# rensortino/DDP-Tutorial

Measured on AMD Instinct MI355X. Metric: images/sec (whole node), ResNet-18 CIFAR-10, higher is better.
Workload: dtype bf16; 1 GPU; model=resnet18, global_batch=8192, image_size=32, num_classes=10, parallelism=dp1, sync_bn=False, hip_graph=False

## Files before the change

mi355x/csrc/conv_mfma.hip:

```cpp
#include "conv_internal.h"

typedef __attribute__((ext_vector_type(8))) _Float16 half8;
typedef __attribute__((ext_vector_type(16))) float f32x16;

namespace {

template <typename T16>
struct Mfma32 {};
template <>
struct Mfma32<__hip_bfloat16> {
  static DEV_INLINE f32x16 run(short8 a, short8 b, f32x16 c) {
    return __builtin_amdgcn_mfma_f32_32x32x16_bf16(a, b, c, 0, 0, 0);
  }
};
template <>
struct Mfma32<__half> {
  static DEV_INLINE f32x16 run(short8 a, short8 b, f32x16 c) {
    return __builtin_amdgcn_mfma_f32_32x32x16_f16((half8)a, (half8)b, c, 0, 0,
                                                  0);
  }
};

struct Sc8 {
  float4v s0, s1, h0, h1;
};

DEV_INLINE Sc8 sc8_load(const float* __restrict__ asc,
                        const float* __restrict__ ash, int c) {
  Sc8 r;
  r.s0 = *reinterpret_cast<const float4v*>(asc + c);
  r.s1 = *reinterpret_cast<const float4v*>(asc + c + 4);
  r.h0 = *reinterpret_cast<const float4v*>(ash + c);
  r.h1 = *reinterpret_cast<const float4v*>(ash + c + 4);
  return r;
}

template <typename T16>
DEV_INLINE short8 scale8(short8 v, const Sc8& sc) {
  short8 o;
#pragma unroll
  for (int u = 0; u < 4; ++u) {
    const float f = s16_to_f32<T16>(v[u]) * sc.s0[u] + sc.h0[u];
    o[u] = f32_to_s16<T16>(fmaxf(f, 0.f));
  }
#pragma unroll
  for (int u = 0; u < 4; ++u) {
    const float f = s16_to_f32<T16>(v[4 + u]) * sc.s1[u] + sc.h1[u];
    o[4 + u] = f32_to_s16<T16>(fmaxf(f, 0.f));
  }
  return o;
}

// ... 107 lines not shown
    if (cc_i == 0) {
      bool va = m_ok;
      long ioff = 0;
      if constexpr (TRANS) {
        const int ph = ih0 + pad - r_;
        const int qw = iw0 + pad - s_;
        const int pp = ph / stride, qq = qw / stride;
        va = va && ph >= 0 && qw >= 0 && (ph % stride) == 0 &&
             (qw % stride) == 0 && pp < Hi && qq < Wi;
        if (va) ioff = (((long)n_ * Hi + pp) * Wi + qq) * CI;
      } else {
        const int ih = ih0 + r_;
        const int iw = iw0 + s_;
        va = va && (unsigned)ih < (unsigned)Hi && (unsigned)iw < (unsigned)Wi;
        if (va) ioff = (((long)n_ * Hi + ih) * Wi + iw) * CI;
      }
      va_tap = va;
      ioff_tap = ioff;
    }
    if (++cc_i == cchunks) {
      cc_i = 0;
      if (++s_i == S) {
        s_i = 0;
        ++r_i;
      }
    }
    const bool va = va_tap;
    const long ioff = ioff_tap;
    const T16* xp = va ? in + ioff + c0 + sa_c : zpage;
#pragma unroll
    for (int i = 0; i < 4; ++i)
      sa[i] = *reinterpret_cast<const short8*>(xp + (va ? 8 * i : 0));
    if constexpr (SCALED) {
      if (va) {
#pragma unroll
        for (int i = 0; i < 4; ++i)
          sa[i] = scale8<T16>(sa[i],
                              sc8_load(asc, ash, c0 + sa_c + 8 * i));
      }
    }
    const T16* wp = wrow + (long)(r_ * S + s_) * b_rs_stride + c0;
#pragma unroll
    for (int i = 0; i < EPT / 8; ++i)
      sb[i] = *reinterpret_cast<const short8*>(wp + 8 * i);
  };

  auto stage = [&]() {
    T16* ldsA = lds;
    T16* ldsB = lds + BM * LDK;
    short* pa = reinterpret_cast<short*>(ldsA + sa_m * LDK + sa_c);
#pragma unroll
    for (int i = 0; i < 4; ++i)
      *reinterpret_cast<short8*>(pa + 8 * i) = sa[i];
    short* pb = reinterpret_cast<short*>(ldsB + sb_n * LDK + sb_c);
#pragma unroll
    for (int i = 0; i < EPT / 8; ++i)
      *reinterpret_cast<short8*>(pb + 8 * i) = sb[i];
  };

  load_step(0);
  for (int j = 0; j < ksteps; ++j) {
    __syncthreads();
    stage();
    __syncthreads();
    if (j + 1 < ksteps) load_step(j + 1);
    const T16* ldsA = lds;
    const T16* ldsB = lds + BM * LDK;
#pragma unroll
    for (int kk = 0; kk < BK; kk += 16) {
      const short8 af = *reinterpret_cast<const short8*>(
          ldsA + (wm + li) * LDK + kk + kh * 8);
#pragma unroll
      for (int tnt = 0; tnt < NT; ++tnt) {
        const short8 bf = *reinterpret_cast<const short8*>(
            ldsB + (tnt * 32 + li) * LDK + kk + kh * 8);
        acc[tnt] = Mfma32<T16>::run(af, bf, acc[tnt]);
      }
    }
  }

  float bv[NT];
  float ssum[NT] = {}, ssq[NT] = {};
#pragma unroll
  for (int tnt = 0; tnt < NT; ++tnt)
    bv[tnt] = has_bias ? bias[k0 + tnt * 32 + li] : 0.f;
#pragma unroll
  for (int reg = 0; reg < 16; ++reg) {
    const int row = (reg & 3) + 8 * (reg >> 2) + 4 * kh;
    const long m_out = bm0 + wm + row;
    if (m_out < Mtot) {
#pragma unroll
      for (int tnt = 0; tnt < NT; ++tnt) {
        float v = acc[tnt][reg] + bv[tnt];
        if constexpr (ADDIN)
          v += F16<T16>::to_f32(addin[m_out * KO + k0 + tnt * 32 + li]);
        if (act == 1) v = fmaxf(v, 0.f);
        if (stats_slab) {
          ssum[tnt] += v;
          ssq[tnt] += v * v;
        }
        out[m_out * KO + k0 + tnt * 32 + li] = F16<T16>::from_f32(v);
      }
    }
  }
  if (stats_slab) {
    constexpr int BNTC = NT * 32;
#pragma unroll
    for (int tnt = 0; tnt < NT; ++tnt) {
      ssum[tnt] += __shfl_xor(ssum[tnt], 32, 64);
      ssq[tnt] += __shfl_xor(ssq[tnt], 32, 64);
    }
    float* lsum = reinterpret_cast<float*>(lds);
    __syncthreads();
    if (kh == 0) {
#pragma unroll
      for (int tnt = 0; tnt < NT; ++tnt) {
        lsum[wave * 2 * BNTC + tnt * 32 + li] = ssum[tnt];
        lsum[wave * 2 * BNTC + BNTC + tnt * 32 + li] = ssq[tnt];
      }
    }
    __syncthreads();
    float* slab =
        stats_slab + ((long)blockIdx.y * gridDim.x + blockIdx.x) * 2 * BNTC;
    for (int t = tid; t < 2 * BNTC; t += 256)
      slab[t] = lsum[t] + lsum[2 * BNTC + t] + lsum[4 * BNTC + t] +
                lsum[6 * BNTC + t];
  }
}

__global__ void conv_stats_partial(const float* __restrict__ slab,
                                   float* __restrict__ out, int gx, int bnt2,
                                   int bpb) {
  const int by = blockIdx.y;
  const int t = threadIdx.x;
  if (t >= bnt2) return;
  const int b0 = blockIdx.x * bpb;
  const int b1 = min(gx, b0 + bpb);
  float acc = 0.f;
  for (int bx = b0; bx < b1; ++bx)
    acc += slab[((long)by * gx + bx) * bnt2 + t];
  out[((long)by * gridDim.x + blockIdx.x) * bnt2 + t] = acc;
}

__global__ void conv_stats_reduce(const float* __restrict__ slab,
                                  float* __restrict__ stats, int gx, int bnt2,
                                  int C, int bx_per_block) {
  const int by = blockIdx.y;
  const int t = threadIdx.x;
  if (t >= bnt2) return;
  float acc = 0.f;
  const int b0 = blockIdx.x * bx_per_block;
  const int b1 = min(gx, b0 + bx_per_block);
  for (int bx = b0; bx < b1; ++bx)
    acc += slab[((long)by * gx + bx) * bnt2 + t];
  const int bnt = bnt2 / 2;
  const int h = t / bnt;
  const int c = by * bnt + (t % bnt);
  stats[h * C + c] = acc;
}

template <typename T16, int NT, bool ADDIN = false>
__global__ __launch_bounds__(256, 2) void conv_dgrad_s2_gemm(
    const T16* __restrict__ dy,
    const T16* __restrict__ wflip,
    const T16* __restrict__ zpage,
    const T16* __restrict__ addin,
    T16* __restrict__ dx,
    const int N, const int P, const int Q, const int KO, const int CI,
    const int H, const int W, const int R, const int S, const int pad) {
  __shared__ T16 lds[BM * LDK + NT * 32 * LDK];
  const int tid = threadIdx.x;
// ... 28 lines not shown
  constexpr int TPR = 256 / BNT;
  constexpr int EPT = BK / TPR;
  const int sb_n = tid / TPR;
  const int sb_c = (tid % TPR) * EPT;

  const int wave = tid >> 6;
  const int lane = tid & 63;
  const int li = lane & 31;
  const int kh = lane >> 5;
  const int wm = wave * 32;
  f32x16 acc[NT] = {};
  short8 sa[4], sb[EPT / 8];

  int cc_i = 0, s_i = 0, r_i = 0;
  bool va_tap = false;
  long ioff_tap = 0, woff_tap = 0;
  auto load_step = [&](int j) {
    (void)j;
    const int c0 = cc_i * BK;
    if (cc_i == 0) {
      const int s_ = s0 + 2 * s_i;
      const int r_ = r0 + 2 * r_i;
      const int dh = ih_ + pad - r_;
      const int dw_ = iw_ + pad - s_;
      const int pp = dh >> 1, qq = dw_ >> 1;
      va_tap = m_ok && dh >= 0 && dw_ >= 0 && pp < P && qq < Q;
      ioff_tap = (((long)n_ * P + pp) * Q + qq) * KO;
      woff_tap = ((long)r_ * S + s_) * CI * (long)KO;
    }
    if (++cc_i == cchunks) {
      cc_i = 0;
      if (++s_i == ns) {
        s_i = 0;
        ++r_i;
      }
    }
    const bool va = va_tap;
    const T16* xp = va ? dy + ioff_tap + c0 + sa_c : zpage;
#pragma unroll
    for (int i = 0; i < 4; ++i)
      sa[i] = *reinterpret_cast<const short8*>(xp + (va ? 8 * i : 0));
    const T16* wp = wflip + woff_tap + (long)(k0 + sb_n) * KO + c0 + sb_c;
#pragma unroll
    for (int i = 0; i < EPT / 8; ++i)
      sb[i] = *reinterpret_cast<const short8*>(wp + 8 * i);
  };
  auto stage = [&]() {
    T16* ldsA = lds;
    T16* ldsB = lds + BM * LDK;
    short* pa_ = reinterpret_cast<short*>(ldsA + sa_m * LDK + sa_c);
#pragma unroll
    for (int i = 0; i < 4; ++i)
      *reinterpret_cast<short8*>(pa_ + 8 * i) = sa[i];
    short* pb_ = reinterpret_cast<short*>(ldsB + sb_n * LDK + sb_c);
#pragma unroll
    for (int i = 0; i < EPT / 8; ++i)
      *reinterpret_cast<short8*>(pb_ + 8 * i) = sb[i];
  };

  if (ksteps > 0) {
    load_step(0);
    for (int j = 0; j < ksteps; ++j) {
      __syncthreads();
      stage();
      __syncthreads();
      if (j + 1 < ksteps) load_step(j + 1);
      const T16* ldsA = lds;
      const T16* ldsB = lds + BM * LDK;
#pragma unroll
      for (int kk = 0; kk < BK; kk += 16) {
        const short8 af = *reinterpret_cast<const short8*>(
            ldsA + (wm + li) * LDK + kk + kh * 8);
#pragma unroll
        for (int tnt = 0; tnt < NT; ++tnt) {
          const short8 bf = *reinterpret_cast<const short8*>(
              ldsB + (tnt * 32 + li) * LDK + kk + kh * 8);
          acc[tnt] = Mfma32<T16>::run(af, bf, acc[tnt]);
        }
      }
    }
  }

  const long m_base = bm0 + wm;
  const int HaWa = Ha * Wa;
  int nn0 = 0, rem0 = 0;
  if (m_base < Mc) {
    nn0 = (int)(m_base / HaWa);
    rem0 = (int)(m_base % HaWa);
  }
#pragma unroll
  for (int reg = 0; reg < 16; ++reg) {
    const int row = (reg & 3) + 8 * (reg >> 2) + 4 * kh;
    const long m_out = m_base + row;
    if (m_out < Mc) {
      int nn = nn0, rem = rem0 + row;
      while (rem >= HaWa) {
        rem -= HaWa;
        ++nn;
      }
      const int ih = 2 * (rem / Wa) + pa;
      const int iw = 2 * (rem - (rem / Wa) * Wa) + pb;
      const long off = (((long)nn * H + ih) * W + iw) * CI;
#pragma unroll
      for (int tnt = 0; tnt < NT; ++tnt) {
        float v = acc[tnt][reg];
        if constexpr (ADDIN)
          v += F16<T16>::to_f32(addin[off + k0 + tnt * 32 + li]);
        dx[off + k0 + tnt * 32 + li] = F16<T16>::from_f32(v);
      }
    }
  }
}

}

void stats_slab_reduce(at::Tensor slab, at::Tensor stats, int gx, int bnt2,
                       int C) {
  const int by = (int)(slab.numel() / ((long)gx * bnt2));
  if (gx > 4096) {
    const int bpb1 = (int)cdiv_l(gx, 1024);
    const int gx2 = (int)cdiv_l(gx, bpb1);
    auto l2 = at::empty({(long)by * gx2 * bnt2}, slab.options());
    launch256(conv_stats_partial, dim3(gx2, by), 0, slab.data_ptr<float>(),
              l2.data_ptr<float>(), gx, bnt2, bpb1);
    slab = l2;
    gx = gx2;
  }
  if (gx > 64) {
    const int bpb2 = (int)cdiv_l(gx, 64);
    const int gx3 = (int)cdiv_l(gx, bpb2);
    auto l3 = at::empty({(long)by * gx3 * bnt2}, slab.options());
    launch256(conv_stats_partial, dim3(gx3, by), 0, slab.data_ptr<float>(),
              l3.data_ptr<float>(), gx, bnt2, bpb2);
    slab = l3;
    gx = gx3;
  }
  launch256(conv_stats_reduce, dim3(1, by), 0, slab.data_ptr<float>(),
            stats.data_ptr<float>(), gx, bnt2, C, gx);
}

constexpr int PCS = 72;

template <typename T16, bool TRANS, bool ADDIN = false, bool SCALED = false>
__global__ __launch_bounds__(256, 2) void conv_patch_gemm(
    const T16* __restrict__ in,
    const T16* __restrict__ wgt,
    const float* __restrict__ bias,
    const T16* __restrict__ addin,
    const float* __restrict__ asc,
    const float* __restrict__ ash,
    T16* __restrict__ out,
    float* __restrict__ stats_slab,
    const int N, const int Hi, const int Wi, const int CI, const int KO,
    const long b_row_stride, const long b_rs_stride, const int act,
    const int has_bias, const int NR) {
  extern __shared__ __attribute__((aligned(16))) char psmem[];
  T16* patch = reinterpret_cast<T16*>(psmem);
  T16* zstub = patch + (long)NR * (Wi + 2) * PCS;
  T16* ldsB = zstub + PCS;

  const int tid = threadIdx.x;
  const long Mtot = (long)N * Hi * Wi;
  const int Wo = Wi, Ho = Hi;
  const long bm0 = (long)blockIdx.x * 128;
  const int k0 = blockIdx.y * 64;
  const long gr0 = bm0 / Wo - 1;

  const int wave = tid >> 6;
  const int lane = tid & 63;
  const int li = lane & 31;
  const int kh = lane >> 5;
  const int wm = wave * 32;

  const long m_lane = bm0 + wm + li;
  const long grl = m_lane / Wo;
  const int p_lane = (int)(grl % Ho);
  const int prow = (int)(grl - gr0);
  const int pcol = (int)(m_lane - grl * Wo) + 1;
  const bool m_ok = m_lane < Mtot;
  const long lane_base = ((long)prow * (Wi + 2) + pcol) * PCS;

  if (tid < 64) zstub[tid] = T16{};

  const int cchunks = CI / BK;
  f32x16 acc[2] = {};

  const int sb_n = tid >> 2;
  const int sb_c = (tid & 3) * 16;
  const T16* wrowB = wgt + (long)(k0 + sb_n) * b_row_stride + sb_c;
  short8 breg[2];
  auto load_b = [&](int tap, int cc) {
    const T16* wp = wrowB + (long)tap * b_rs_stride + cc * BK;
    breg[0] = *reinterpret_cast<const short8*>(wp);
    breg[1] = *reinterpret_cast<const short8*>(wp + 8);
  };
  auto stage_b = [&]() {
    short* pb = reinterpret_cast<short*>(ldsB + sb_n * LDK + sb_c);
    *reinterpret_cast<short8*>(pb) = breg[0];
    *reinterpret_cast<short8*>(pb + 8) = breg[1];
  };

  load_b(0, 0);

  for (int cc = 0; cc < cchunks; ++cc) {
    __syncthreads();
    const int ngroups = NR * (Wi + 2) * (BK / 8);
    for (int i0f = tid; i0f < ngroups; i0f += 4 * 256) {
      const T16* srcs[4];
      short8 vals[4];
      int dsts[4], gs[4];
      bool ok[4];
#pragma unroll
      for (int b = 0; b < 4; ++b) {
        const int i = i0f + b * 256;
        const int g = i % (BK / 8);
        const int ce = i / (BK / 8);
        const int col = ce % (Wi + 2);
        const int row = ce / (Wi + 2);
        const long gr = gr0 + row;
        const int iw = col - 1;
        gs[b] = g;
        dsts[b] = i < ngroups ? (row * (Wi + 2) + col) * PCS + g * 8 : -1;
        ok[b] = i < ngroups && gr >= 0 && gr < (long)N * Ho &&
                (unsigned)iw < (unsigned)Wi;
        const long nn = ok[b] ? gr / Ho : 0;
        const long pp = ok[b] ? gr % Ho : 0;
        srcs[b] = ok[b]
                      ? in + ((nn * Hi + pp) * Wi + iw) * CI + cc * BK + g * 8
                      : zstub;
      }
#pragma unroll
      for (int b = 0; b < 4; ++b)
        vals[b] = *reinterpret_cast<const short8*>(srcs[b]);
#pragma unroll
      for (int b = 0; b < 4; ++b) {
        if (dsts[b] < 0) break;
        short8 v = vals[b];
        if (!ok[b]) v = short8{};
        if constexpr (SCALED) {
          if (ok[b])
            v = scale8<T16>(v, sc8_load(asc, ash, cc * BK + gs[b] * 8));
        }
        *reinterpret_cast<short8*>(patch + dsts[b]) = v;
      }
    }
    __syncthreads();

#pragma unroll
    for (int r = 0; r < 3; ++r) {
      const int pv = TRANS ? p_lane + 1 - r : p_lane + r - 1;
      const bool rv = m_ok && (unsigned)pv < (unsigned)Ho;
#pragma unroll
      for (int s = 0; s < 3; ++s) {
        const int tap = r * 3 + s;
        const long off = TRANS
                             ? ((long)(1 - r) * (Wi + 2) + (1 - s)) * PCS
                             : ((long)(r - 1) * (Wi + 2) + (s - 1)) * PCS;
        const T16* abase = rv ? patch + lane_base + off : zstub;
        __syncthreads();
        stage_b();
        __syncthreads();
        if (tap < 8)
          load_b(tap + 1, cc);
        else if (cc + 1 < cchunks)
          load_b(0, cc + 1);
#pragma unroll
        for (int kk = 0; kk < 4; ++kk) {
          const short8 af = *reinterpret_cast<const short8*>(
              abase + kk * 16 + kh * 8);
          const short8 b0 = *reinterpret_cast<const short8*>(
              ldsB + li * LDK + kk * 16 + kh * 8);
          const short8 b1 = *reinterpret_cast<const short8*>(
              ldsB + (32 + li) * LDK + kk * 16 + kh * 8);
          acc[0] = Mfma32<T16>::run(af, b0, acc[0]);
          acc[1] = Mfma32<T16>::run(af, b1, acc[1]);
        }
      }
    }
  }

  float bv[2];
  bv[0] = has_bias ? bias[k0 + li] : 0.f;
  bv[1] = has_bias ? bias[k0 + 32 + li] : 0.f;
  float ssum[2] = {}, ssq[2] = {};
#pragma unroll
  for (int reg = 0; reg < 16; ++reg) {
    const int row = (reg & 3) + 8 * (reg >> 2) + 4 * kh;
    const long m_out = bm0 + wm + row;
    if (m_out < Mtot) {
#pragma unroll
      for (int t2 = 0; t2 < 2; ++t2) {
        float v = acc[t2][reg] + bv[t2];
        if constexpr (ADDIN)
          v += F16<T16>::to_f32(addin[m_out * KO + k0 + t2 * 32 + li]);
        if (act == 1) v = fmaxf(v, 0.f);
        if (stats_slab) {
          ssum[t2] += v;
          ssq[t2] += v * v;
        }
        out[m_out * KO + k0 + t2 * 32 + li] = F16<T16>::from_f32(v);
      }
    }
  }
  if (stats_slab) {
#pragma unroll
    for (int t2 = 0; t2 < 2; ++t2) {
      ssum[t2] += __shfl_xor(ssum[t2], 32, 64);
      ssq[t2] += __shfl_xor(ssq[t2], 32, 64);
    }
    float* lsum = reinterpret_cast<float*>(psmem);
    __syncthreads();
    if (kh == 0) {
#pragma unroll
      for (int t2 = 0; t2 < 2; ++t2) {
        lsum[wave * 128 + t2 * 32 + li] = ssum[t2];
        lsum[wave * 128 + 64 + t2 * 32 + li] = ssq[t2];
      }
    }
    __syncthreads();
    float* slab =
        stats_slab + ((long)blockIdx.y * gridDim.x + blockIdx.x) * 2 * 64;
    for (int t = tid; t < 2 * 64; t += 256)
      slab[t] = lsum[t] + lsum[128 + t] + lsum[256 + t] + lsum[384 + t];
  }
}


namespace {

constexpr int WGM = 64;
constexpr int LDM = 72;

template <typename T16, int KT, bool SCALED = false, bool KMIN = false>
__global__ __launch_bounds__(256, SCALED ? 4 : 2) void conv_wgrad_mfma_kernel(
    const T16* __restrict__ x,
    const T16* __restrict__ dy,
    const float* __restrict__ asc,
    const float* __restrict__ ash,
    float* __restrict__ dw,
    const int N, const int Hi, const int Wi, const int CI, const int KO,
    const int Ho, const int Wo, const int R, const int S, const int stride,
    const int pad, const long m_per_chunk, const int nchunks) {
  __shared__ T16 lds[(KT + 64) * LDM];

  const int tid = threadIdx.x;
  const long Mtot = (long)N * Ho * Wo;
  const int k0 = blockIdx.x * KT;
  const int cchunks = CI / BK;
  const int c0 = (blockIdx.y % cchunks) * BK;
  const int s_ = (blockIdx.y / cchunks) % S;
  const int r_ = blockIdx.y / (cchunks * S);
  const long m_begin = (long)blockIdx.z * m_per_chunk;
  const long m_end = min(Mtot, m_begin + m_per_chunk);

  const bool do_dy = tid < 2 * KT;
  const bool do_x = KT == 64 ? tid >= 128 : tid < 128;
  const int t = do_dy ? tid : 0;
  constexpr int KG = KT / 8;
  const int sm = KMIN ? (t / KG) * 4 : (t & 15) * 4;
  const int sk = KMIN ? (t % KG) * 8 : (t >> 4) * 8;
  const int tx = tid & 127;
  const int smx = KMIN ? (tx >> 3) * 4 : (tx & 15) * 4;
  const int skx = KMIN ? (tx & 7) * 8 : (tx >> 4) * 8;

  const int wave = tid >> 6;
  const int lane = tid & 63;
  const int li = lane & 31;
  const int kh = lane >> 5;
  constexpr int NJ = KT / 64;
// ... 861 lines not shown
  at::Tensor zp = conv_zero_page(in);
  at::Tensor slab;
  if (present(stats))
    slab = at::empty({(long)grid.y * grid.x * 2 * nt * 32},
                     in.options().dtype(at::kFloat));
  DISPATCH_16(in, T16, {
    auto go = [&](auto kern) {
      launch256(kern, grid, 0, (const T16*)in.data_ptr(),
                (const T16*)wgt.data_ptr(), f32_or_null(bias),
                (const T16*)zp.data_ptr(),
                present(addin) ? (const T16*)addin.data_ptr() : nullptr, asc,
                ash, (T16*)out.data_ptr(), f32_or_null(slab), N, Hi, Wi, CI,
                KO, Ho, Wo, R, S, stride, pad, b_row_stride, b_rs_stride, act,
                present(bias));
    };
    if (genc)
      go(conv_gather_gemm<T16, false, true, 2>);
    else
      pick<4, 2>(nt, [&](auto NT) {
        if (trans)
          pick<true, false>(present(addin), [&](auto ADDIN) {
            go(conv_gather_gemm<T16, true, false, decltype(NT)::value,
                                decltype(ADDIN)::value>);
          });
        else
          pick<true, false>(asc != nullptr, [&](auto SCALED) {
            go(conv_gather_gemm<T16, false, false, decltype(NT)::value, false,
                                decltype(SCALED)::value>);
          });
      });
  });
  if (slab.defined()) stats_slab_reduce(slab, stats, grid.x, 2 * nt * 32, KO);
}

struct PatchGeom {
  int NR;
  size_t smem;
};
PatchGeom patch_geom(int W) {
  const int NR = (W + 126) / W + 3;
  return {NR, ((size_t)NR * (W + 2) * PCS + PCS + 64 * LDK) * 2};
}

void patch_gemm_launch(bool trans, const at::Tensor& in,
                       const at::Tensor& wgt, const at::Tensor& bias,
                       const at::Tensor& addin, const float* asc,
                       const float* ash, at::Tensor& out,
                       const at::Tensor& stats, long b_row_stride,
                       long b_rs_stride, long act) {
  const int N = in.size(0), Hi = in.size(1), Wi = in.size(2), CI = in.size(3);
  const int KO = out.size(3);
  const long M = (long)N * Hi * Wi;
  const PatchGeom pg = patch_geom(Wi);
  dim3 grid((unsigned)cdiv_l(M, 128), KO / 64);
  at::Tensor slab;
  if (present(stats))
    slab = at::empty({(long)grid.y * grid.x * 128},
                     in.options().dtype(at::kFloat));
  DISPATCH_16(in, T16, {
    auto go = [&](auto kern) {
      launch256(kern, grid, pg.smem, (const T16*)in.data_ptr(),
                (const T16*)wgt.data_ptr(), f32_or_null(bias),
                present(addin) ? (const T16*)addin.data_ptr() : nullptr, asc,
                ash, (T16*)out.data_ptr(), f32_or_null(slab), N, Hi, Wi, CI,
                KO, b_row_stride, b_rs_stride, act, present(bias), pg.NR);
    };
    if (trans)
      pick<true, false>(present(addin), [&](auto ADDIN) {
        go(conv_patch_gemm<T16, true, decltype(ADDIN)::value>);
      });
    else
      pick<true, false>(asc != nullptr, [&](auto SCALED) {
        go(conv_patch_gemm<T16, false, false, decltype(SCALED)::value>);
      });
  });
  if (slab.defined()) stats_slab_reduce(slab, stats, grid.x, 128, KO);
}

void dgrad_s2_launch(const at::Tensor& dy, const at::Tensor& wflip,
                     at::Tensor& dx, const at::Tensor& addin, long R, long S,
                     long pad) {
  const int N = dy.size(0), P = dy.size(1), Q = dy.size(2), KO = dy.size(3);
  const int H = dx.size(1), W = dx.size(2), CI = dx.size(3);
  const long Mmax = (long)N * ((H + 1) / 2) * ((W + 1) / 2);
  const bool wide = CI % 128 == 0 && cdiv_l(Mmax, BM) * (CI / 128) * 4 >= 1024;
  const int nt = wide ? 4 : 2;
  dim3 grid((unsigned)cdiv_l(Mmax, BM), CI / (nt * 32), 4);
  at::Tensor zp = conv_zero_page(dy);
  DISPATCH_16(dy, T16, {
    pick<4, 2>(nt, [&](auto NT) {
      pick<true, false>(present(addin), [&](auto ADDIN) {
        launch256(conv_dgrad_s2_gemm<T16, decltype(NT)::value,
                                     decltype(ADDIN)::value>,
                  grid, 0, (const T16*)dy.data_ptr(),
                  (const T16*)wflip.data_ptr(), (const T16*)zp.data_ptr(),
                  present(addin) ? (const T16*)addin.data_ptr() : nullptr,
                  (T16*)dx.data_ptr(), N, P, Q, KO, CI, H, W, R, S, pad);
      });
    });
  });
}

}

void conv_fwd_mfma_genc_launch(at::Tensor x, at::Tensor wpad, at::Tensor bias,
                               at::Tensor y, long R, long S, long stride,
// ... 45 lines not shown
```

mi355x/csrc/stem_mfma.hip:

```cpp
#include "conv_internal.h"

typedef __attribute__((ext_vector_type(8))) _Float16 half8_s;
typedef __attribute__((ext_vector_type(16))) float f32x16_s;

namespace {

template <int R_>
struct StemGeo {};
template <>
struct StemGeo<7> {
  static constexpr int SROW = 24, SKG = 192, VALID = 21;
};
template <>
struct StemGeo<3> {
  static constexpr int SROW = 16, SKG = 64, VALID = 9;
};

constexpr int SLDK = 64 + 8;
constexpr int SLDM = 72;

template <typename T16>
struct SMfma {};
template <>
struct SMfma<__hip_bfloat16> {
  static DEV_INLINE f32x16_s run(short8 a, short8 b, f32x16_s c) {
    return __builtin_amdgcn_mfma_f32_32x32x16_bf16(a, b, c, 0, 0, 0);
  }
};
template <>
struct SMfma<__half> {
  static DEV_INLINE f32x16_s run(short8 a, short8 b, f32x16_s c) {
    return __builtin_amdgcn_mfma_f32_32x32x16_f16((half8_s)a, (half8_s)b, c,
                                                  0, 0, 0);
  }
};

template <typename T16>
struct G8 {
  const T16* src;
  long base;
  int e0, jj;
  unsigned char fast, row_ok;
};

template <typename T16, int R_, int STRIDE_>
DEV_INLINE void g8_plan(G8<T16>& g, const T16* __restrict__ x,
                        const T16* __restrict__ zpage, int n, int p, int q,
                        int kg0, int H, int W3, int pad, bool m_ok) {
  constexpr int SROW = StemGeo<R_>::SROW;
  const int r = kg0 / SROW;
  g.jj = kg0 - r * SROW;
  const int ih = STRIDE_ * p - pad + r;
// ... 35 lines not shown
    const float* __restrict__ bias, const T16* __restrict__ zpage,
    T16* __restrict__ y, const int N, const int H, const int W,
    const int KO, const int Ho, const int Wo, const int pad, const int act,
    const int has_bias) {
  constexpr int SKG = StemGeo<R_>::SKG;
  __shared__ T16 lds[128 * SLDK + 64 * SLDK];
  const int tid = threadIdx.x;
  const long Mtot = (long)N * Ho * Wo;
  const long bm0 = (long)blockIdx.x * 128;
  const int k0 = blockIdx.y * 64;
  const int W3 = 3 * W;

  const int sa_m = tid >> 1;
  const int sa_c = (tid & 1) * 32;
  const long m_a = bm0 + sa_m;
  const bool m_ok = m_a < Mtot;
  int n_ = 0, p_ = 0, q_ = 0;
  if (m_ok) {
    n_ = (int)(m_a / ((long)Ho * Wo));
    const int pq = (int)(m_a % ((long)Ho * Wo));
    p_ = pq / Wo;
    q_ = pq % Wo;
  }
  const int sb_n = tid >> 2;
  const int sb_c = (tid & 3) * 16;

  const int wave = tid >> 6;
  const int lane = tid & 63;
  const int li = lane & 31;
  const int kh = lane >> 5;
  const int wm = wave * 32;
  f32x16_s acc[2] = {};

  short8 sa[4], sb[2];
  auto load_step = [&](int j) {
    G8<T16> g[4];
#pragma unroll
    for (int i = 0; i < 4; ++i)
      g8_plan<T16, R_, STRIDE_>(g[i], x, zpage, n_, p_, q_,
                                j * 64 + sa_c + 8 * i, H, W3, pad, m_ok);
#pragma unroll
    for (int i = 0; i < 4; ++i)
      sa[i] = *reinterpret_cast<const short8*>(g[i].src);
#pragma unroll
    for (int i = 0; i < 4; ++i) sa[i] = g8_fix<T16, R_>(g[i], sa[i], x, W3);
    const T16* wp = w24 + (long)(k0 + sb_n) * SKG + j * 64 + sb_c;
    sb[0] = *reinterpret_cast<const short8*>(wp);
    sb[1] = *reinterpret_cast<const short8*>(wp + 8);
  };
  auto stage = [&]() {
    short* pa = reinterpret_cast<short*>(lds + sa_m * SLDK + sa_c);
#pragma unroll
    for (int i = 0; i < 4; ++i) *reinterpret_cast<short8*>(pa + 8 * i) = sa[i];
    short* pb =
        reinterpret_cast<short*>(lds + 128 * SLDK + sb_n * SLDK + sb_c);
    *reinterpret_cast<short8*>(pb) = sb[0];
    *reinterpret_cast<short8*>(pb + 8) = sb[1];
  };

  load_step(0);
  for (int j = 0; j < SKG / 64; ++j) {
    __syncthreads();
    stage();
    __syncthreads();
    if (j + 1 < SKG / 64) load_step(j + 1);
    const T16* ldsA = lds;
    const T16* ldsB = lds + 128 * SLDK;
#pragma unroll
    for (int kk = 0; kk < 64; kk += 16) {
      const short8 af = *reinterpret_cast<const short8*>(
          ldsA + (wm + li) * SLDK + kk + kh * 8);
      const short8 b0 = *reinterpret_cast<const short8*>(
          ldsB + li * SLDK + kk + kh * 8);
      const short8 b1 = *reinterpret_cast<const short8*>(
          ldsB + (32 + li) * SLDK + kk + kh * 8);
      acc[0] = SMfma<T16>::run(af, b0, acc[0]);
      acc[1] = SMfma<T16>::run(af, b1, acc[1]);
    }
  }

  float bv[2];
  bv[0] = has_bias ? bias[k0 + li] : 0.f;
  bv[1] = has_bias ? bias[k0 + 32 + li] : 0.f;
#pragma unroll
  for (int reg = 0; reg < 16; ++reg) {
    const int row = (reg & 3) + 8 * (reg >> 2) + 4 * kh;
    const long m_out = bm0 + wm + row;
    if (m_out < Mtot) {
#pragma unroll
      for (int t2 = 0; t2 < 2; ++t2) {
        float v = acc[t2][reg] + bv[t2];
        if (act == 1) v = fmaxf(v, 0.f);
        y[m_out * KO + k0 + t2 * 32 + li] = F16<T16>::from_f32(v);
      }
    }
  }
}

template <typename T16, int R_, int STRIDE_>
__global__ __launch_bounds__(256, 2) void conv_fwd_stem_strip(
    const T16* __restrict__ x,
    const T16* __restrict__ w24,
    const float* __restrict__ bias,
    float* __restrict__ stats_slab,
    T16* __restrict__ y, const int N,
    const int H, const int W, const int KO, const int Ho, const int Wo,
    const int pad, const int act, const int has_bias, const int nrows,
    const int sstride) {
  constexpr int SROW = StemGeo<R_>::SROW;
  constexpr int SKG = StemGeo<R_>::SKG;
  constexpr int VALID = StemGeo<R_>::VALID;
  extern __shared__ __attribute__((aligned(16))) char ssmem[];
  T16* strip = reinterpret_cast<T16*>(ssmem);
  T16* ldsB = strip + (long)(nrows + 1) * sstride;
  const int tid = threadIdx.x;
  const int W3 = 3 * W;
  const long Mimg = (long)Ho * Wo;
  const long bm0 = (long)blockIdx.x * 128;
  const int n = (int)(bm0 / Mimg);
  const long bmi = bm0 - (long)n * Mimg;
  const int p0 = (int)(bmi / Wo);
  const int ih0 = STRIDE_ * p0 - pad;
  const int k0 = blockIdx.y * 64;

  const int off3 = 3 * pad;
  const int nv8 = (W3 + 7) / 8;
  for (int t = tid; t < nrows * nv8; t += 256) {
    const int rr = t / nv8;
    const int j8 = (t - rr * nv8) * 8;
    const int ih = ih0 + rr;
    T16* dst = strip + (long)rr * sstride + off3 + j8;
    if ((unsigned)ih < (unsigned)H && j8 + 8 <= W3) {
      *reinterpret_cast<short8*>(dst) =
          *reinterpret_cast<const short8*>(x + ((long)n * H + ih) * W3 + j8);
    } else {
      const T16 z{};
#pragma unroll
      for (int u = 0; u < 8; ++u)
        dst[u] = (j8 + u < W3 && (unsigned)ih < (unsigned)H)
                     ? x[((long)n * H + ih) * W3 + j8 + u]
                     : z;
    }
  }
  {
    const int nz = sstride - W3;
    const T16 z{};
    for (int t = tid; t < nrows * nz; t += 256) {
      const int rr = t / nz;
      const int e = t - rr * nz;
      strip[(long)rr * sstride + (e < off3 ? e : W3 + e)] = z;
    }
    for (int t = tid; t < sstride; t += 256)
      strip[(long)nrows * sstride + t] = z;
  }
  for (int e = tid * 8; e < 64 * SKG; e += 256 * 8) {
    const int row = e / SKG, col = e - row * SKG;
    *reinterpret_cast<short8*>(
        reinterpret_cast<short*>(ldsB + row * (SKG + 8) + col)) =
        *reinterpret_cast<const short8*>(w24 + (long)(k0 + row) * SKG + col);
  }
  __syncthreads();

  const int wave = tid >> 6;
  const int lane = tid & 63;
  const int li = lane & 31;
  const int kh = lane >> 5;
  const int wm = wave * 32;
  const long mi = bmi + wm + li;
  const int p_lane = (int)(mi / Wo);
  const int q_lane = (int)(mi - (long)p_lane * Wo);
  const int rr_base = STRIDE_ * (p_lane - p0);
  const int ebase = 3 * STRIDE_ * q_lane;
  f32x16_s acc[2] = {};

#pragma unroll
  for (int slice = 0; slice < SKG / 16; ++slice) {
    const int kg0 = slice * 16 + kh * 8;
    const int r = kg0 / SROW;
    const int jj = kg0 - r * SROW;
    const int rr = r < R_ ? rr_base + r : nrows;
    const short* ap = reinterpret_cast<const short*>(
        strip + (long)rr * sstride + ebase + jj);
    short8 af;
#pragma unroll
    for (int u2 = 0; u2 < 4; ++u2) {
      int v32;
      __builtin_memcpy(&v32, ap + 2 * u2, 4);
      __builtin_memcpy(reinterpret_cast<char*>(&af) + 4 * u2, &v32, 4);
    }
    if (jj > VALID - 8) {
#pragma unroll
      for (int u = 0; u < 8; ++u)
        if (jj + u >= VALID) af[u] = 0;
    }
    const short8 b0 = *reinterpret_cast<const short8*>(
        ldsB + li * (SKG + 8) + slice * 16 + kh * 8);
    const short8 b1 = *reinterpret_cast<const short8*>(
        ldsB + (32 + li) * (SKG + 8) + slice * 16 + kh * 8);
    acc[0] = SMfma<T16>::run(af, b0, acc[0]);
    acc[1] = SMfma<T16>::run(af, b1, acc[1]);
  }

  float bv[2];
  bv[0] = has_bias ? bias[k0 + li] : 0.f;
  bv[1] = has_bias ? bias[k0 + 32 + li] : 0.f;
  float ssum[2] = {}, ssq[2] = {};
  const long Mtot = (long)N * Mimg;
#pragma unroll
  for (int reg = 0; reg < 16; ++reg) {
    const int row = (reg & 3) + 8 * (reg >> 2) + 4 * kh;
    const long m_out = bm0 + wm + row;
    if (m_out < Mtot) {
#pragma unroll
      for (int t2 = 0; t2 < 2; ++t2) {
        float v = acc[t2][reg] + bv[t2];
        if (act == 1) v = fmaxf(v, 0.f);
        if (stats_slab) {
          ssum[t2] += v;
          ssq[t2] += v * v;
        }
        y[m_out * KO + k0 + t2 * 32 + li] = F16<T16>::from_f32(v);
      }
    }
  }
  if (stats_slab) {
#pragma unroll
    for (int t2 = 0; t2 < 2; ++t2) {
      ssum[t2] += __shfl_xor(ssum[t2], 32, 64);
      ssq[t2] += __shfl_xor(ssq[t2], 32, 64);
    }
    float* lsum = reinterpret_cast<float*>(ssmem);
    __syncthreads();
    if (kh == 0) {
#pragma unroll
      for (int t2 = 0; t2 < 2; ++t2) {
        lsum[wave * 128 + t2 * 32 + li] = ssum[t2];
        lsum[wave * 128 + 64 + t2 * 32 + li] = ssq[t2];
      }
    }
    __syncthreads();
    float* slab =
        stats_slab + ((long)blockIdx.y * gridDim.x + blockIdx.x) * 2 * 64;
    for (int t = tid; t < 2 * 64; t += 256)
      slab[t] = lsum[t] + lsum[128 + t] + lsum[256 + t] + lsum[384 + t];
  }
}

template <typename T16, int R_, int STRIDE_>
__global__ __launch_bounds__(256, 2) void conv_wgrad_stem_gemm(
    const T16* __restrict__ x,
    const T16* __restrict__ dy,
    const T16* __restrict__ zpage,
    float* __restrict__ dw,
    const int N, const int H, const int W, const int KO, const int Ho,
    const int Wo, const int pad, const long m_per_chunk) {
  constexpr int SROW = StemGeo<R_>::SROW;
  constexpr int SKG = StemGeo<R_>::SKG;
  constexpr int VALID = StemGeo<R_>::VALID;
  constexpr int NJ = SKG / 64;
  __shared__ T16 lds[(64 + SKG) * SLDM];
  const int tid = threadIdx.x;
  const long Mtot = (long)N * Ho * Wo;
  const int k0 = blockIdx.x * 64;
  const long m_begin = (long)blockIdx.y * m_per_chunk;
  const long m_end = min(Mtot, m_begin + m_per_chunk);
  const int W3 = 3 * W;

  const bool do_dy = tid < 128;
  const bool do_x = tid >= 128;
  const int t = do_dy ? tid : 0;
  const int sm = (t & 15) * 4;
  const int sk = (t >> 4) * 8;
  const int tx = tid & 127;
  const int smx = (tx & 15) * 4;
  const int gx0 = (tx >> 4) * NJ;

  const int wave = tid >> 6;
  const int lane = tid & 63;
  const int li = lane & 31;
  const int kh = lane >> 5;
  const int i0 = (wave & 1) * 32;
  const int j0 = (wave >> 1) * 32;

  f32x16_s acc[NJ] = {};

  int dn = 0, dp = 0, dq = 0;
  {
    const long m_first = m_begin + smx;
    dn = (int)(m_first / ((long)Ho * Wo));
    const int pq = (int)(m_first % ((long)Ho * Wo));
// ... 100 lines not shown
#pragma unroll
  for (int jt = 0; jt < NJ; ++jt) {
    const int kg = j0 + jt * 64 + li;
    const int r = kg / SROW;
    const int jj = kg - r * SROW;
    if (jj < VALID && r < R_) {
      const int s = jj / 3, c = jj - s * 3;
#pragma unroll
      for (int reg = 0; reg < 16; ++reg) {
        const int i = (reg & 3) + 8 * (reg >> 2) + 4 * kh;
        slab[(((long)(k0 + i0 + i) * 3 + c) * R_ + r) * R_ + s] =
            acc[jt][reg];
      }
    }
  }
}

}


template <int R_>
static at::Tensor stem_wpad(const at::Tensor& w) {
  constexpr int SROW = StemGeo<R_>::SROW;
  constexpr int SKG = StemGeo<R_>::SKG;
  const long KO = w.size(0);
  auto valid = w.narrow(1, 0, 3 * R_ * R_).reshape({KO, R_, 3 * R_});
  auto padded = at::constant_pad_nd(valid, {0, SROW - 3 * R_}, 0);
  return at::constant_pad_nd(padded.reshape({KO, R_ * SROW}),
                             {0, SKG - R_ * SROW}, 0)
      .contiguous();
}

template <int R_, int STRIDE_>
static bool fwd_stem_gemm_impl(at::Tensor x, at::Tensor w, at::Tensor bias,
                               at::Tensor y, long pad, long act,
                               at::Tensor stats) {
  constexpr int SKG = StemGeo<R_>::SKG;
  const int N = x.size(0), H = x.size(1), W = x.size(2);
  const int KO = w.size(0);
  const int Ho = y.size(1), Wo = y.size(2);
  TORCH_CHECK(KO % 64 == 0, "stem GEMM expects KO % 64 == 0");
  auto w24 = stem_wpad<R_>(w);
  const long M = (long)N * Ho * Wo;
  dim3 grid((unsigned)cdiv_l(M, 128), KO / 64);
  const int has_bias = bias.numel() > 0;
  static const bool strip_on = EnvKnob("MI355X_STEM_STRIP").on();
  const long Mimg = (long)Ho * Wo;
  if (strip_on && Mimg % 128 == 0) {
    const int pspan = (int)((127 / Wo) + 1);
    const int nrows = STRIDE_ * (pspan - 1) + R_;
    const int sstride = (3 * W + 6 * (int)pad + 8 + 3) & ~3;
    const size_t smem =
        ((size_t)(nrows + 1) * sstride + 64 * (SKG + 8)) * x.element_size();
    if (smem <= 150 * 1024) {
      const bool want_stats = stats.defined() && stats.numel() > 0;
      at::Tensor slab;
      float* slab_p = nullptr;
      if (want_stats) {
        slab = at::empty({(long)grid.y * grid.x * 128},
                         x.options().dtype(at::kFloat));
        slab_p = slab.data_ptr<float>();
      }
      DISPATCH_16(x, T16, {
        launch256(conv_fwd_stem_strip<T16, R_, STRIDE_>, grid, smem,
                  (const T16*)x.data_ptr(), (const T16*)w24.data_ptr(),
                  has_bias ? bias.data_ptr<float>() : nullptr, slab_p,
                  (T16*)y.data_ptr(), N, H, W, KO, Ho, Wo, pad, act, has_bias,
                  nrows, sstride);
      });
      if (slab_p)
        stats_slab_reduce(slab, stats, grid.x, 128, KO);
      return want_stats;
    }
  }
  at::Tensor zp = conv_zero_page(x);
  DISPATCH_16(x, T16, {
    launch256(conv_fwd_stem_gemm<T16, R_, STRIDE_>, grid, 0,
              (const T16*)x.data_ptr(), (const T16*)w24.data_ptr(),
              has_bias ? bias.data_ptr<float>() : nullptr,
              (const T16*)zp.data_ptr(), (T16*)y.data_ptr(), N, H, W, KO, Ho,
              Wo, pad, act, has_bias);
  });
  return false;
}

bool conv_fwd_stem_gemm_launch(at::Tensor x, at::Tensor w, at::Tensor bias,
                               at::Tensor y, long pad, long act,
                               at::Tensor stats, long R, long stride) {
  if (R == 7 && stride == 2)
    return fwd_stem_gemm_impl<7, 2>(x, w, bias, y, pad, act, stats);
  TORCH_CHECK(R == 3 && stride == 1, "stem GEMM: unsupported (R, stride)");
  return fwd_stem_gemm_impl<3, 1>(x, w, bias, y, pad, act, stats);
}

template <int R_, int STRIDE_>
static void wgrad_stem_gemm_impl(at::Tensor x, at::Tensor dy, at::Tensor dw,
                                 long pad) {
  const int N = x.size(0), H = x.size(1), W = x.size(2);
  const int Ho = dy.size(1), Wo = dy.size(2), KO = dy.size(3);
  TORCH_CHECK(KO % 64 == 0, "stem wgrad GEMM expects KO % 64 == 0");
  const long M = (long)N * Ho * Wo;
  const long E = (long)KO * 3 * R_ * R_;
  const SplitPlan sp = split_plan(M, std::min<long>(512, cdiv_l(M, 4096)));
  auto part = at::empty({sp.n * E}, x.options().dtype(at::kFloat));
  at::Tensor zp = conv_zero_page(x);
  dim3 grid(KO / 64, (unsigned)sp.n);
// ... 17 lines not shown
```

Before: 138,300 images/sec.

## Stage conv GEMM epilogue through LDS for coalesced 16-byte row stores

Output-channel rows of the B tile are permuted so each lane's MFMA accumulators cover adjacent channels. The epilogue then packs results into per-wave LDS tiles and flushes full rows with 16-byte vector stores, and residual add-in inputs are fetched the same way. This replaces scattered 2-byte global loads and stores across the forward, dgrad, patch and stem conv kernels. It costs an extra block barrier, LDS round trips and reuse of the A/B LDS buffer, and bias and stats indexing are remapped to the new channel order.

```diff
diff --git a/mi355x/csrc/conv_epilogue.h b/mi355x/csrc/conv_epilogue.h
--- /dev/null
+++ b/mi355x/csrc/conv_epilogue.h
@@ -0,0 +1,88 @@
+#pragma once
+
+#include "common.h"
+
+typedef __attribute__((ext_vector_type(2))) short short2v;
+
+template <int NT, int ROWS = 32>
+struct EpiTile {
+  static constexpr int RS = NT * 32 + 8;
+  static constexpr int LPR = NT * 4;
+  static constexpr int RPI = 64 / LPR;
+  static constexpr int NIT = ROWS / RPI;
+  static constexpr int WAVE = ROWS * RS;
+  static constexpr int BYTES = 4 * WAVE * 2;
+};
+
+template <int NT>
+struct EpiPack {};
+template <>
+struct EpiPack<2> {
+  typedef short2v type;
+};
+template <>
+struct EpiPack<4> {
+  typedef short4v type;
+};
+
+DEV_INLINE void epi_wave_sync() {
+  asm volatile("s_waitcnt lgkmcnt(0)" ::: "memory");
+}
+
+template <int NT>
+DEV_INLINE int epi_brow(int n) {
+  return (n % NT) * 32 + n / NT;
+}
+
+DEV_INLINE int epi_acc_row(int reg, int kh) {
+  return (reg & 3) + 8 * (reg >> 2) + 4 * kh;
+}
+
+template <int NT>
+DEV_INLINE int epi_io_row(int it, int lane) {
+  return it * EpiTile<NT>::RPI + lane / EpiTile<NT>::LPR;
+}
+
+template <typename T16, int NT, int ROWS = 32>
+DEV_INLINE void epi_fetch(short* wl, const T16* __restrict__ g, int lane,
+                          const long (&roff)[EpiTile<NT, ROWS>::NIT]) {
+  using E = EpiTile<NT, ROWS>;
+  const int c = (lane % E::LPR) * 8;
+  short8 v[E::NIT];
+#pragma unroll
+  for (int it = 0; it < E::NIT; ++it)
+    v[it] = roff[it] >= 0
+                ? *reinterpret_cast<const short8*>(g + roff[it] + c)
+                : short8{};
+#pragma unroll
+  for (int it = 0; it < E::NIT; ++it)
+    *reinterpret_cast<short8*>(wl + epi_io_row<NT>(it, lane) * E::RS + c) =
+        v[it];
+}
+
+template <int NT>
+DEV_INLINE typename EpiPack<NT>::type epi_get(const short* wl, int row,
+                                              int li) {
+  return *reinterpret_cast<const typename EpiPack<NT>::type*>(
+      wl + row * EpiTile<NT>::RS + li * NT);
+}
+
+template <int NT>
+DEV_INLINE void epi_put(short* wl, int row, int li,
+                        typename EpiPack<NT>::type h) {
+  *reinterpret_cast<typename EpiPack<NT>::type*>(
+      wl + row * EpiTile<NT>::RS + li * NT) = h;
+}
+
+template <typename T16, int NT, int ROWS = 32>
+DEV_INLINE void epi_flush(const short* wl, T16* __restrict__ g, int lane,
+                          const long (&roff)[EpiTile<NT, ROWS>::NIT]) {
+  using E = EpiTile<NT, ROWS>;
+  const int c = (lane % E::LPR) * 8;
+#pragma unroll
+  for (int it = 0; it < E::NIT; ++it) {
+    const short8 v = *reinterpret_cast<const short8*>(
+        wl + epi_io_row<NT>(it, lane) * E::RS + c);
+    if (roff[it] >= 0) *reinterpret_cast<short8*>(g + roff[it] + c) = v;
+  }
+}
diff --git a/mi355x/csrc/conv_mfma.hip b/mi355x/csrc/conv_mfma.hip
--- a/mi355x/csrc/conv_mfma.hip
+++ b/mi355x/csrc/conv_mfma.hip
@@ -1,3 +1,4 @@
+#include "conv_epilogue.h"
 #include "conv_internal.h"
 
 typedef __attribute__((ext_vector_type(8))) _Float16 half8;
@@ -211,7 +212,8 @@
 #pragma unroll
     for (int i = 0; i < 4; ++i)
       *reinterpret_cast<short8*>(pa + 8 * i) = sa[i];
-    short* pb = reinterpret_cast<short*>(ldsB + sb_n * LDK + sb_c);
+    short* pb =
+        reinterpret_cast<short*>(ldsB + epi_brow<NT>(sb_n) * LDK + sb_c);
 #pragma unroll
     for (int i = 0; i < EPT / 8; ++i)
       *reinterpret_cast<short8*>(pb + 8 * i) = sb[i];
@@ -238,30 +240,47 @@
     }
   }
 
+  using E = EpiTile<NT>;
+  static_assert(sizeof(lds) >= E::BYTES, "epilogue tile must fit the A/B LDS");
+  short* wl = reinterpret_cast<short*>(lds) + wave * E::WAVE;
+  long roff[E::NIT];
+#pragma unroll
+  for (int it = 0; it < E::NIT; ++it) {
+    const long m = bm0 + wm + epi_io_row<NT>(it, lane);
+    roff[it] = m < Mtot ? m * KO + k0 : -1;
+  }
+  __syncthreads();
+  if constexpr (ADDIN) {
+    epi_fetch<T16, NT>(wl, addin, lane, roff);
+    epi_wave_sync();
+  }
   float bv[NT];
   float ssum[NT] = {}, ssq[NT] = {};
 #pragma unroll
   for (int tnt = 0; tnt < NT; ++tnt)
-    bv[tnt] = has_bias ? bias[k0 + tnt * 32 + li] : 0.f;
+    bv[tnt] = has_bias ? bias[k0 + li * NT + tnt] : 0.f;
 #pragma unroll
   for (int reg = 0; reg < 16; ++reg) {
-    const int row = (reg & 3) + 8 * (reg >> 2) + 4 * kh;
-    const long m_out = bm0 + wm + row;
-    if (m_out < Mtot) {
+    const int row = epi_acc_row(reg, kh);
+    typename EpiPack<NT>::type h = {};
+    if (bm0 + wm + row < Mtot) {
+      if constexpr (ADDIN) h = epi_get<NT>(wl, row, li);
 #pragma unroll
       for (int tnt = 0; tnt < NT; ++tnt) {
         float v = acc[tnt][reg] + bv[tnt];
-        if constexpr (ADDIN)
-          v += F16<T16>::to_f32(addin[m_out * KO + k0 + tnt * 32 + li]);
+        if constexpr (ADDIN) v += s16_to_f32<T16>(h[tnt]);
         if (act == 1) v = fmaxf(v, 0.f);
         if (stats_slab) {
           ssum[tnt] += v;
           ssq[tnt] += v * v;
         }
-        out[m_out * KO + k0 + tnt * 32 + li] = F16<T16>::from_f32(v);
-      }
-    }
-  }
+        h[tnt] = f32_to_s16<T16>(v);
+      }
+    }
+    epi_put<NT>(wl, row, li, h);
+  }
+  epi_wave_sync();
+  epi_flush<T16, NT>(wl, out, lane, roff);
   if (stats_slab) {
     constexpr int BNTC = NT * 32;
 #pragma unroll
@@ -274,8 +293,8 @@
     if (kh == 0) {
 #pragma unroll
       for (int tnt = 0; tnt < NT; ++tnt) {
-        lsum[wave * 2 * BNTC + tnt * 32 + li] = ssum[tnt];
-        lsum[wave * 2 * BNTC + BNTC + tnt * 32 + li] = ssq[tnt];
+        lsum[wave * 2 * BNTC + li * NT + tnt] = ssum[tnt];
+        lsum[wave * 2 * BNTC + BNTC + li * NT + tnt] = ssq[tnt];
       }
     }
     __syncthreads();
@@ -410,7 +429,8 @@
 #pragma unroll
     for (int i = 0; i < 4; ++i)
       *reinterpret_cast<short8*>(pa_ + 8 * i) = sa[i];
-    short* pb_ = reinterpret_cast<short*>(ldsB + sb_n * LDK + sb_c);
+    short* pb_ =
+        reinterpret_cast<short*>(ldsB + epi_brow<NT>(sb_n) * LDK + sb_c);
 #pragma unroll
     for (int i = 0; i < EPT / 8; ++i)
       *reinterpret_cast<short8*>(pb_ + 8 * i) = sb[i];
@@ -439,6 +459,9 @@
     }
   }
 
+  using E = EpiTile<NT>;
+  static_assert(sizeof(lds) >= E::BYTES, "epilogue tile must fit the A/B LDS");
+  short* wl = reinterpret_cast<short*>(lds) + wave * E::WAVE;
   const long m_base = bm0 + wm;
   const int HaWa = Ha * Wa;
   int nn0 = 0, rem0 = 0;
@@ -446,11 +469,12 @@
     nn0 = (int)(m_base / HaWa);
     rem0 = (int)(m_base % HaWa);
   }
-#pragma unroll
-  for (int reg = 0; reg < 16; ++reg) {
-    const int row = (reg & 3) + 8 * (reg >> 2) + 4 * kh;
-    const long m_out = m_base + row;
-    if (m_out < Mc) {
+  long roff[E::NIT];
+#pragma unroll
+  for (int it = 0; it < E::NIT; ++it) {
+    const int row = epi_io_row<NT>(it, lane);
+    roff[it] = -1;
+    if (m_base + row < Mc) {
       int nn = nn0, rem = rem0 + row;
       while (rem >= HaWa) {
         rem -= HaWa;
@@ -458,16 +482,29 @@
       }
       const int ih = 2 * (rem / Wa) + pa;
       const int iw = 2 * (rem - (rem / Wa) * Wa) + pb;
-      const long off = (((long)nn * H + ih) * W + iw) * CI;
-#pragma unroll
-      for (int tnt = 0; tnt < NT; ++tnt) {
-        float v = acc[tnt][reg];
-        if constexpr (ADDIN)
-          v += F16<T16>::to_f32(addin[off + k0 + tnt * 32 + li]);
-        dx[off + k0 + tnt * 32 + li] = F16<T16>::from_f32(v);
-      }
-    }
-  }
+      roff[it] = (((long)nn * H + ih) * W + iw) * CI + k0;
+    }
+  }
+  __syncthreads();
+  if constexpr (ADDIN) {
+    epi_fetch<T16, NT>(wl, addin, lane, roff);
+    epi_wave_sync();
+  }
+#pragma unroll
+  for (int reg = 0; reg < 16; ++reg) {
+    const int row = epi_acc_row(reg, kh);
+    typename EpiPack<NT>::type h = {};
+    if constexpr (ADDIN) h = epi_get<NT>(wl, row, li);
+#pragma unroll
+    for (int tnt = 0; tnt < NT; ++tnt) {
+      float v = acc[tnt][reg];
+      if constexpr (ADDIN) v += s16_to_f32<T16>(h[tnt]);
+      h[tnt] = f32_to_s16<T16>(v);
+    }
+    epi_put<NT>(wl, row, li, h);
+  }
+  epi_wave_sync();
+  epi_flush<T16, NT>(wl, dx, lane, roff);
 }
 
 }
@@ -512,6 +549,7 @@
     const int N, const int Hi, const int Wi, const int CI, const int KO,
     const long b_row_stride, const long b_rs_stride, const int act,
     const int has_bias, const int NR) {
+  constexpr bool ROWST = ADDIN;
   extern __shared__ __attribute__((aligned(16))) char psmem[];
   T16* patch = reinterpret_cast<T16*>(psmem);
   T16* zstub = patch + (long)NR * (Wi + 2) * PCS;
@@ -553,7 +591,8 @@
     breg[1] = *reinterpret_cast<const short8*>(wp + 8);
   };
   auto stage_b = [&]() {
-    short* pb = reinterpret_cast<short*>(ldsB + sb_n * LDK + sb_c);
+    short* pb = reinterpret_cast<short*>(
+        ldsB + (ROWST ? epi_brow<2>(sb_n) : sb_n) * LDK + sb_c);
     *reinterpret_cast<short8*>(pb) = breg[0];
     *reinterpret_cast<short8*>(pb + 8) = breg[1];
   };
@@ -637,26 +676,62 @@
     }
   }
 
+  const int ch[2] = {ROWST ? 2 * li : li, ROWST ? 2 * li + 1 : 32 + li};
   float bv[2];
-  bv[0] = has_bias ? bias[k0 + li] : 0.f;
-  bv[1] = has_bias ? bias[k0 + 32 + li] : 0.f;
+  bv[0] = has_bias ? bias[k0 + ch[0]] : 0.f;
+  bv[1] = has_bias ? bias[k0 + ch[1]] : 0.f;
   float ssum[2] = {}, ssq[2] = {};
-#pragma unroll
-  for (int reg = 0; reg < 16; ++reg) {
-    const int row = (reg & 3) + 8 * (reg >> 2) + 4 * kh;
-    const long m_out = bm0 + wm + row;
-    if (m_out < Mtot) {
-#pragma unroll
-      for (int t2 = 0; t2 < 2; ++t2) {
-        float v = acc[t2][reg] + bv[t2];
-        if constexpr (ADDIN)
-          v += F16<T16>::to_f32(addin[m_out * KO + k0 + t2 * 32 + li]);
-        if (act == 1) v = fmaxf(v, 0.f);
-        if (stats_slab) {
-          ssum[t2] += v;
-          ssq[t2] += v * v;
+  if constexpr (ROWST) {
+    using E = EpiTile<2>;
+    short* wl = reinterpret_cast<short*>(psmem) + wave * E::WAVE;
+    long roff[E::NIT];
+#pragma unroll
+    for (int it = 0; it < E::NIT; ++it) {
+      const long m = bm0 + wm + epi_io_row<2>(it, lane);
+      roff[it] = m < Mtot ? m * KO + k0 : -1;
+    }
+    __syncthreads();
+    if constexpr (ADDIN) {
+      epi_fetch<T16, 2>(wl, addin, lane, roff);
+      epi_wave_sync();
+    }
+#pragma unroll
+    for (int reg = 0; reg < 16; ++reg) {
+      const int row = epi_acc_row(reg, kh);
+      short2v h = {};
+      if (bm0 + wm + row < Mtot) {
+        if constexpr (ADDIN) h = epi_get<2>(wl, row, li);
+#pragma unroll
+        for (int t2 = 0; t2 < 2; ++t2) {
+          float v = acc[t2][reg] + bv[t2];
+          if constexpr (ADDIN) v += s16_to_f32<T16>(h[t2]);
+          if (act == 1) v = fmaxf(v, 0.f);
+          if (stats_slab) {
+            ssum[t2] += v;
+            ssq[t2] += v * v;
+          }
+          h[t2] = f32_to_s16<T16>(v);
         }
-        out[m_out * KO + k0 + t2 * 32 + li] = F16<T16>::from_f32(v);
+      }
+      epi_put<2>(wl, row, li, h);
+    }
+    epi_wave_sync();
+    epi_flush<T16, 2>(wl, out, lane, roff);
+  } else {
+#pragma unroll
+    for (int reg = 0; reg < 16; ++reg) {
+      const long m_out = bm0 + wm + epi_acc_row(reg, kh);
+      if (m_out < Mtot) {
+#pragma unroll
+        for (int t2 = 0; t2 < 2; ++t2) {
+          float v = acc[t2][reg] + bv[t2];
+          if (act == 1) v = fmaxf(v, 0.f);
+          if (stats_slab) {
+            ssum[t2] += v;
+            ssq[t2] += v * v;
+          }
+          out[m_out * KO + k0 + ch[t2]] = F16<T16>::from_f32(v);
+        }
       }
     }
   }
@@ -671,8 +746,8 @@
     if (kh == 0) {
 #pragma unroll
       for (int t2 = 0; t2 < 2; ++t2) {
-        lsum[wave * 128 + t2 * 32 + li] = ssum[t2];
-        lsum[wave * 128 + 64 + t2 * 32 + li] = ssq[t2];
+        lsum[wave * 128 + ch[t2]] = ssum[t2];
+        lsum[wave * 128 + 64 + ch[t2]] = ssq[t2];
       }
     }
     __syncthreads();
@@ -1640,6 +1715,8 @@
   const int KO = out.size(3);
   const long M = (long)N * Hi * Wi;
   const PatchGeom pg = patch_geom(Wi);
+  TORCH_CHECK(pg.smem >= (size_t)EpiTile<2>::BYTES,
+              "patch LDS smaller than the epilogue's staged tile");
   dim3 grid((unsigned)cdiv_l(M, 128), KO / 64);
   at::Tensor slab;
   if (present(stats))
diff --git a/mi355x/csrc/stem_mfma.hip b/mi355x/csrc/stem_mfma.hip
--- a/mi355x/csrc/stem_mfma.hip
+++ b/mi355x/csrc/stem_mfma.hip
@@ -1,3 +1,4 @@
+#include "conv_epilogue.h"
 #include "conv_internal.h"
 
 typedef __attribute__((ext_vector_type(8))) _Float16 half8_s;
@@ -139,8 +140,8 @@
     short* pa = reinterpret_cast<short*>(lds + sa_m * SLDK + sa_c);
 #pragma unroll
     for (int i = 0; i < 4; ++i) *reinterpret_cast<short8*>(pa + 8 * i) = sa[i];
-    short* pb =
-        reinterpret_cast<short*>(lds + 128 * SLDK + sb_n * SLDK + sb_c);
+    short* pb = reinterpret_cast<short*>(lds + 128 * SLDK +
+                                         epi_brow<2>(sb_n) * SLDK + sb_c);
     *reinterpret_cast<short8*>(pb) = sb[0];
     *reinterpret_cast<short8*>(pb + 8) = sb[1];
   };
@@ -166,22 +167,32 @@
     }
   }
 
+  using E = EpiTile<2>;
+  static_assert(sizeof(lds) >= E::BYTES, "epilogue tile must fit the A/B LDS");
+  short* wl = reinterpret_cast<short*>(lds) + wave * E::WAVE;
+  long roff[E::NIT];
+#pragma unroll
+  for (int it = 0; it < E::NIT; ++it) {
+    const long m = bm0 + wm + epi_io_row<2>(it, lane);
+    roff[it] = m < Mtot ? m * KO + k0 : -1;
+  }
   float bv[2];
-  bv[0] = has_bias ? bias[k0 + li] : 0.f;
-  bv[1] = has_bias ? bias[k0 + 32 + li] : 0.f;
+  bv[0] = has_bias ? bias[k0 + 2 * li] : 0.f;
+  bv[1] = has_bias ? bias[k0 + 2 * li + 1] : 0.f;
+  __syncthreads();
 #pragma unroll
   for (int reg = 0; reg < 16; ++reg) {
-    const int row = (reg & 3) + 8 * (reg >> 2) + 4 * kh;
-    const long m_out = bm0 + wm + row;
-    if (m_out < Mtot) {
-#pragma unroll
-      for (int t2 = 0; t2 < 2; ++t2) {
-        float v = acc[t2][reg] + bv[t2];
-        if (act == 1) v = fmaxf(v, 0.f);
-        y[m_out * KO + k0 + t2 * 32 + li] = F16<T16>::from_f32(v);
-      }
-    }
-  }
+    short2v h;
+#pragma unroll
+    for (int t2 = 0; t2 < 2; ++t2) {
+      float v = acc[t2][reg] + bv[t2];
+      if (act == 1) v = fmaxf(v, 0.f);
+      h[t2] = f32_to_s16<T16>(v);
+    }
+    epi_put<2>(wl, epi_acc_row(reg, kh), li, h);
+  }
+  epi_wave_sync();
+  epi_flush<T16, 2>(wl, y, lane, roff);
 }
 
 template <typename T16, int R_, int STRIDE_>
@@ -243,7 +254,8 @@
   for (int e = tid * 8; e < 64 * SKG; e += 256 * 8) {
     const int row = e / SKG, col = e - row * SKG;
     *reinterpret_cast<short8*>(
-        reinterpret_cast<short*>(ldsB + row * (SKG + 8) + col)) =
+        reinterpret_cast<short*>(ldsB + epi_brow<2>(row) * (SKG + 8) +
+                                 col)) =
         *reinterpret_cast<const short8*>(w24 + (long)(k0 + row) * SKG + col);
   }
   __syncthreads();
@@ -288,27 +300,46 @@
     acc[1] = SMfma<T16>::run(af, b1, acc[1]);
   }
 
+  using E = EpiTile<2, 16>;
+  short* wl = reinterpret_cast<short*>(ssmem) + wave * E::WAVE;
   float bv[2];
-  bv[0] = has_bias ? bias[k0 + li] : 0.f;
-  bv[1] = has_bias ? bias[k0 + 32 + li] : 0.f;
+  bv[0] = has_bias ? bias[k0 + 2 * li] : 0.f;
+  bv[1] = has_bias ? bias[k0 + 2 * li + 1] : 0.f;
   float ssum[2] = {}, ssq[2] = {};
   const long Mtot = (long)N * Mimg;
 #pragma unroll
-  for (int reg = 0; reg < 16; ++reg) {
-    const int row = (reg & 3) + 8 * (reg >> 2) + 4 * kh;
-    const long m_out = bm0 + wm + row;
-    if (m_out < Mtot) {
-#pragma unroll
-      for (int t2 = 0; t2 < 2; ++t2) {
-        float v = acc[t2][reg] + bv[t2];
-        if (act == 1) v = fmaxf(v, 0.f);
-        if (stats_slab) {
-          ssum[t2] += v;
-          ssq[t2] += v * v;
+  for (int half = 0; half < 2; ++half) {
+    long roff[E::NIT];
+#pragma unroll
+    for (int it = 0; it < E::NIT; ++it) {
+      const long m = bm0 + wm + half * 16 + epi_io_row<2>(it, lane);
+      roff[it] = m < Mtot ? m * KO + k0 : -1;
+    }
+    if (half == 0)
+      __syncthreads();
+    else
+      epi_wave_sync();
+#pragma unroll
+    for (int r8 = 0; r8 < 8; ++r8) {
+      const int reg = half * 8 + r8;
+      const int row = epi_acc_row(reg, kh);
+      short2v h = {};
+      if (bm0 + wm + row < Mtot) {
+#pragma unroll
+        for (int t2 = 0; t2 < 2; ++t2) {
+          float v = acc[t2][reg] + bv[t2];
+          if (act == 1) v = fmaxf(v, 0.f);
+          if (stats_slab) {
+            ssum[t2] += v;
+            ssq[t2] += v * v;
+          }
+          h[t2] = f32_to_s16<T16>(v);
         }
-        y[m_out * KO + k0 + t2 * 32 + li] = F16<T16>::from_f32(v);
-      }
-    }
+      }
+      epi_put<2>(wl, row - half * 16, li, h);
+    }
+    epi_wave_sync();
+    epi_flush<T16, 2, 16>(wl, y, lane, roff);
   }
   if (stats_slab) {
 #pragma unroll
@@ -321,8 +352,8 @@
     if (kh == 0) {
 #pragma unroll
       for (int t2 = 0; t2 < 2; ++t2) {
-        lsum[wave * 128 + t2 * 32 + li] = ssum[t2];
-        lsum[wave * 128 + 64 + t2 * 32 + li] = ssq[t2];
+        lsum[wave * 128 + 2 * li + t2] = ssum[t2];
+        lsum[wave * 128 + 64 + 2 * li + t2] = ssq[t2];
       }
     }
     __syncthreads();
@@ -529,6 +560,7 @@
     const int sstride = (3 * W + 6 * (int)pad + 8 + 3) & ~3;
     const size_t smem =
         ((size_t)(nrows + 1) * sstride + 64 * (SKG + 8)) * x.element_size();
+    static_assert(64 * (SKG + 8) * 2 >= EpiTile<2, 16>::BYTES);
     if (smem <= 150 * 1024) {
       const bool want_stats = stats.defined() && stats.numel() > 0;
       at::Tensor slab;
```

Result: faster. 142,900 images/sec (median of 6 runs) (+3.4%).
